# renmengye/rec-attend-public

Hardware: AMD Instinct MI355X
Metric: instance-timesteps/sec, full_model forward 512x512 T=16 (whole job; pipelined throughput: 8 batches in flight per GPU, fill and drain of the pipeline inside the timed region; config.lone_batch_* = one sync-bracketed forward) (higher is better)
Workload: dtype f32; 1 GPU; cfg2: CVPPP-arch full_model eval forward, 512x512, T=16, B=8 per GPU, y_out+s_out; arch=cvppp, H=512, W=512, T=16, batch_per_gpu=8, global_batch=8, parallelism=batch-sharded x1, no collective, ranks_in_communicator=1, hip_graph=True, tile_tickets=False, batches_in_flight=8, pipeline_slots=4, batches_per_launch=2, input=resident in HBM, output=left in HBM

## Files before the change

### rec-attend-public_amd/csrc/ra_ctrl_split.hip

```cpp
#include <cstdlib>
#include <type_traits>

#include "ra_common.h"
#include "ra_ctrl_parts.h"

namespace ra {
namespace ctrl2 {

typedef float f32x4 __attribute__((ext_vector_type(4)));
typedef unsigned long long u64;

constexpr int kP = 16;
constexpr int kThreads = 256;
constexpr int kMaxFeatRegs = 96;
constexpr unsigned kSpinLimit = 4000000u;
constexpr int kMaxResidentWgs = 224;

struct Layout {
  int us, gs, K, NL;
  size_t lstm_w, lstm_b;
  size_t gh_w[8], gh_b[8];
  size_t gl_w, gl_b;
  size_t slice;
  size_t cmlp;
  size_t cm_w[8], cm_b[8];
  int cm_in[8], cm_out[8];
  size_t total;
  int n_hidden;
};

__host__ __device__ inline Layout layout(const ra_ctrl_desc &d) {
  Layout L;
  L.us = d.hid / kP;
  L.gs = ceil_div(d.G, kP);
  L.K = d.Cf + d.hid;
  L.NL = 4 * L.us;
  L.n_hidden = d.n_gmlp - 1;
  size_t off = 0;
  L.lstm_w = off;
  off += (size_t)L.K * L.NL;
  L.lstm_b = off;
  off += L.NL;
  for (int l = 0; l < L.n_hidden; ++l) {
    L.gh_w[l] = off;
    off += (size_t)d.hid * L.us;
    L.gh_b[l] = off;
    off += L.us;
  }
  L.gl_w = off;
  off += (size_t)d.hid * L.gs;
  L.gl_b = off;
  off += L.gs;
  L.slice = round_up((int)off, 4);
  off = L.slice * kP;
  L.cmlp = off;
  for (int l = 0; l < d.n_cmlp; ++l) {
    L.cm_in[l] = (l == 0) ? d.hid : d.mlp_dim;
    L.cm_out[l] = (l == d.n_cmlp - 1) ? 9 : d.mlp_dim;
    L.cm_w[l] = off;
    off += (size_t)L.cm_in[l] * L.cm_out[l];
    L.cm_b[l] = off;
    off += L.cm_out[l];
  }
  L.total = off;
  return L;
}

__host__ __device__ inline size_t granules_per_image(const ra_ctrl_desc &d) {
  const Layout L = layout(d);
  return (size_t)d.iters * (d.hid + (size_t)L.n_hidden * d.hid + (size_t)kP * L.gs);
}
__host__ __device__ inline size_t ws_words_per_image(const ra_ctrl_desc &d) {
  return 2 + 2 * granules_per_image(d);
}

__host__ inline size_t lds_bytes(const ra_ctrl_desc &d) {
  const Layout L = layout(d);
  return (L.slice + 4 * (size_t)kThreads + round_up(L.K, 4) + d.hid + round_up(kP * L.gs, 4) + 64) * sizeof(float);
}

__host__ inline int supported(const ra_ctrl_desc &d) {
  if (d.hid % kP || d.hid > kThreads || d.Cf <= 0 || kThreads % d.Cf || d.n_gmlp < 1 ||
      d.n_gmlp > 8 || d.n_cmlp < 1 || d.n_cmlp > 8 || d.G <= 0 || d.G > 4096 || d.iters <= 0 ||
      d.mlp_dim > kThreads)
    return 0;
  if (kThreads % (d.hid / kP) || kThreads % (4 * (d.hid / kP))) return 0;
  if ((size_t)d.G * d.Cf > (size_t)kMaxFeatRegs * kThreads) return 0;
  if (4 * layout(d).us > kThreads) return 0;
  return lds_bytes(d) <= 160 * 1024;
}

typedef unsigned u32x2g __attribute__((ext_vector_type(2)));
template <bool XL>
struct Exchange {
  u64 *gran;
  __amdgpu_buffer_rsrc_t rs;
  unsigned tag;
  int err = 0;

  __device__ __forceinline__ Exchange(unsigned *wsb, size_t granules)
      : gran(reinterpret_cast<u64 *>(wsb + 2)),
        rs(__builtin_amdgcn_make_buffer_rsrc(gran, 0, (int)(granules * 8), 0x00020000)),
        tag(wsb[0] + 1u) {}

  __device__ __forceinline__ void publish(size_t idx, float v) const {
    if constexpr (XL)
      __builtin_amdgcn_raw_buffer_store_b64(u32x2g{__float_as_uint(v), tag}, rs, (int)idx * 8, 0, 0);
    else
      __hip_atomic_store(gran + idx, ((u64)tag << 32) | (u64)__float_as_uint(v), __ATOMIC_RELAXED, __HIP_MEMORY_SCOPE_AGENT);
  }

  __device__ __forceinline__ u32x2g load(size_t idx) const {
    if constexpr (XL) {
      return __builtin_amdgcn_raw_buffer_load_b64(rs, (int)idx * 8, 0, (int)0x80000001u);
    } else {
      const u64 x = __hip_atomic_load(gran + idx, __ATOMIC_RELAXED, __HIP_MEMORY_SCOPE_AGENT);
      return u32x2g{(unsigned)x, (unsigned)(x >> 32)};
    }
  }

  template <int INFLIGHT, class Store>
  __device__ __forceinline__ void poll(size_t first, int total, Store store) {
    for (int base = 0; base < total; base += kThreads * INFLIGHT) {
      unsigned pending = 0;
#pragma unroll
      for (int j = 0; j < INFLIGHT; ++j)
        if (base + threadIdx.x + kThreads * j < total) pending |= 1u << j;
      unsigned spins = 0;
      while (pending) {
        u32x2g x[INFLIGHT];
#pragma unroll
        for (int j = 0; j < INFLIGHT; ++j)
          if (pending & (1u << j)) x[j] = load(first + base + threadIdx.x + kThreads * j);
#pragma unroll
        for (int j = 0; j < INFLIGHT; ++j)
          if ((pending & (1u << j)) && x[j].y == tag) {
            store(base + threadIdx.x + kThreads * j, __uint_as_float(x[j].x));
            pending &= ~(1u << j);
          }
        if (pending) {
          if (++spins > kSpinLimit) {
            err = 1;
            break;
          }
          __builtin_amdgcn_s_sleep(1);
        }
      }
    }
    __syncthreads();
  }

  template <int INFLIGHT>
  __device__ __forceinline__ void gather(size_t first, int n, int nimg, float *dst, int stride) {
    poll<INFLIGHT>(first, n * nimg, [&](int e, float v) {
      const int i = e / n, c = e - i * n;
      dst[i * stride + c] = v;
    });
  }
};

__device__ __forceinline__ void fill_slice(float *W, const float *__restrict__ wp, int p, const Layout &L) {
  const int t = threadIdx.x;
  const f32x4 *src = reinterpret_cast<const f32x4 *>(wp + (size_t)p * L.slice);
  f32x4 *dst = reinterpret_cast<f32x4 *>(W);
  const int n4 = (int)(L.slice / 4);
  constexpr int U = 16;
  for (int e0 = t; e0 < n4; e0 += kThreads * U) {
    f32x4 tmp[U];
#pragma unroll
    for (int u = 0; u < U; ++u) {
      const int e = e0 + u * kThreads;
      tmp[u] = src[e < n4 ? e : n4 - 1];
    }
#pragma unroll
    for (int u = 0; u < U; ++u) {
      const int e = e0 + u * kThreads;
      if (e < n4) dst[e] = tmp[u];
    }
  }
}

__device__ float block_reduce(float v, bool is_max, float *red4) {
#pragma unroll
  for (int o = 32; o > 0; o >>= 1) {
    const float other = __shfl_xor(v, o);
    v = is_max ? fmaxf(v, other) : v + other;
  }
  __syncthreads();
  if ((threadIdx.x & 63) == 0) red4[threadIdx.x >> 6] = v;
  __syncthreads();
  const float a = red4[0], b = red4[1], c = red4[2], d = red4[3];
  return is_max ? fmaxf(fmaxf(a, b), fmaxf(c, d)) : (a + b) + (c + d);
}

__device__ inline void slice_gemv(const float *W, int ncol, const float *x, int k0, int K, float *red) {
  const int t = threadIdx.x;
  const int parts = kThreads / ncol;
  const int col = t % ncol, part = t / ncol;
  float acc0 = 0.0f, acc1 = 0.0f;
  int k = k0 + part;
#pragma unroll 4
  for (; k + parts < K; k += 2 * parts) {
    acc0 += x[k] * W[(size_t)k * ncol + col];
    acc1 += x[k + parts] * W[(size_t)(k + parts) * ncol + col];
  }
  if (k < K) acc0 += x[k] * W[(size_t)k * ncol + col];
  red[part * ncol + col] = acc0 + acc1;
  __syncthreads();
}

__device__ inline int any_gemv(const float *Wm, int n, const float *x, int K, float *red, int *ncol_out) {
  const int t = threadIdx.x;
  int ncol = 1;
  while (ncol < n) ncol <<= 1;
  const int parts = kThreads / ncol;
  const int col = t % ncol, part = t / ncol;
  float acc = 0.0f;
  if (col < n)
    for (int k = part; k < K; k += parts) acc += x[k] * Wm[(size_t)k * n + col];
  red[part * ncol + col] = acc;
  __syncthreads();
  *ncol_out = ncol;
  return parts;
}

__device__ __forceinline__ void finish_image(const ra_ctrl_desc &d, const Layout &L, const float *__restrict__ wp, const float *h,
                                             float *o1, float *o2, float *scratch, int b, float *h_last, float *ctrl_out,
                                             float *attn) {
  const int t = threadIdx.x;
  const float *in = h;
  for (int l = 0; l < d.n_cmlp; ++l) {
    const int N = L.cm_out[l], Kin = L.cm_in[l];
    const float *Wc = wp + L.cm_w[l], *bc = wp + L.cm_b[l];
    const bool last = (l == d.n_cmlp - 1);
    int ncol;
    const int parts = any_gemv(Wc, N, in, Kin, scratch, &ncol);
    if (t < N) {
      float a = bc[t];
      for (int q = 0; q < parts; ++q) a += scratch[q * ncol + t];
      o1[t] = last ? a : fmaxf(a, 0.0f);
    }
    __syncthreads();
    in = o1;
    float *tmp = o1;
    o1 = o2;
    o2 = tmp;
  }
  const float *co = in;
  if (t < d.hid && h_last) h_last[(size_t)b * d.hid + t] = h[t];
  if (t < 9 && ctrl_out) ctrl_out[(size_t)b * 9 + t] = co[t];
  if (t == 0 && attn) store_attn_record(d, co, attn + (size_t)b * RA_ATTN_STRIDE);
}

__device__ inline void publish(u64 *g, unsigned tag, float v) {
  __hip_atomic_store(g, ((u64)tag << 32) | (u64)__float_as_uint(v), __ATOMIC_RELAXED,
                     __HIP_MEMORY_SCOPE_AGENT);
}

__device__ inline void gather(const u64 *g, int n, unsigned tag, float *dst, int *err) {
  for (int i = threadIdx.x; i < n; i += kThreads) {
    unsigned spins = 0;
    u64 x;
    while (true) {
      x = __hip_atomic_load(g + i, __ATOMIC_RELAXED, __HIP_MEMORY_SCOPE_AGENT);
      if ((unsigned)(x >> 32) == tag) break;
      if (++spins > kSpinLimit) {
        *err = 1;
        break;
      }
      __builtin_amdgcn_s_sleep(1);
    }
    dst[i] = __uint_as_float((unsigned)x);
  }
  __syncthreads();
}

__device__ inline void publish_l2(__amdgpu_buffer_rsrc_t r, int idx, unsigned tag, float v) {
  __builtin_amdgcn_raw_buffer_store_b64(u32x2g{__float_as_uint(v), tag}, r, idx * 8, 0, 0);
}
__device__ inline void gather_l2(__amdgpu_buffer_rsrc_t r, int first, int n, unsigned tag, float *dst, int *err) {
  for (int i = threadIdx.x; i < n; i += kThreads) {
    unsigned spins = 0;
    u32x2g x;
    while (true) {
      x = __builtin_amdgcn_raw_buffer_load_b64(r, (first + i) * 8, 0, (int)0x80000001u);
      if (x.y == tag) break;
      if (++spins > kSpinLimit) {
        *err = 1;
        break;
      }
      __builtin_amdgcn_s_sleep(1);
    }
    dst[i] = __uint_as_float(x.x);
  }
  __syncthreads();
}

template <int FR, bool XL = false>
__global__ __launch_bounds__(kThreads) void controller_split_kernel(
    const ra_ctrl_desc d, const float *feat, const float *__restrict__ wp, float *h_last,
    float *ctrl_out, float *gmaps, float *attn, unsigned *ws, int *status, int prio, int B, unsigned *tickets) {
  raise_prio(prio);
  extern __shared__ __attribute__((aligned(16))) float smem[];
  const Layout L = layout(d);
  const int t = threadIdx.x;
  int p = blockIdx.x, b = blockIdx.y;
  if constexpr (XL) {
    unsigned *role_sh = reinterpret_cast<unsigned *>(smem);
    const int x = xcc_id(), share = kP * ((B + 7) >> 3);
    if (t == 0) *role_sh = ticket_draw(tickets + x * kTicketPoolStride) % (unsigned)share;
    __syncthreads();
    const int role = (int)*role_sh;
    __syncthreads();
    p = role % kP;
    b = x + 8 * (role / kP);
    if (b >= B) return;
  }
  const int G = d.G, Cf = d.Cf, hid = d.hid, us = L.us, gs = L.gs, K = L.K;
  const int Gx = kP * gs;
  float *W = smem;
  float *red = W + L.slice;
  float *xh = red + 4 * kThreads;
  float *va = xh + round_up(K, 4);
  float *gm = va + hid;
  float *red4 = gm + round_up(Gx, 4);
  unsigned *wsb = ws + (size_t)b * ws_words_per_image(d);
  const unsigned tag = wsb[0] + 1u;
  u64 *gran = reinterpret_cast<u64 *>(wsb + 2);
  const __amdgpu_buffer_rsrc_t grs = __builtin_amdgcn_make_buffer_rsrc(gran, 0, (int)(granules_per_image(d) * 8), 0x00020000);
  int err = 0;
  auto pub = [&](size_t idx, float v) {
    if constexpr (XL) publish_l2(grs, (int)idx, tag, v);
    else publish(gran + idx, tag, v);
  };
  auto gat = [&](size_t first, int n, float *dst) {
    if constexpr (XL) gather_l2(grs, (int)first, n, tag, dst, &err);
    else gather(gran + first, n, tag, dst, &err);
  };

  {
    const f32x4 *src = reinterpret_cast<const f32x4 *>(wp + (size_t)p * L.slice);
    f32x4 *dst = reinterpret_cast<f32x4 *>(W);
    const int n4 = (int)(L.slice / 4);
    constexpr int U = 16;
    for (int e0 = t; e0 < n4; e0 += kThreads * U) {
      f32x4 tmp[U];
#pragma unroll
      for (int u = 0; u < U; ++u) {
        const int e = e0 + u * kThreads;
        tmp[u] = src[e < n4 ? e : n4 - 1];
      }
#pragma unroll
      for (int u = 0; u < U; ++u) {
        const int e = e0 + u * kThreads;
        if (e < n4) dst[e] = tmp[u];
      }
    }
  }
  float fr[FR];
  const float *fsrc = feat + (size_t)b * G * Cf;
#pragma unroll
  for (int i = 0; i < FR; ++i) {
    const int e = t + kThreads * i;
    fr[i] = (e < G * Cf) ? fsrc[e] : 0.0f;
  }
  for (int e = t; e < hid; e += kThreads) xh[Cf + e] = 0.0f;
  for (int g = t; g < Gx; g += kThreads) gm[g] = (g < G) ? 1.0f / (float)G : 0.0f;
  float cst = 0.0f;
  __syncthreads();

  size_t goff = 0;
  for (int it = 0; it < d.iters; ++it) {
    if (gmaps && p == 0)
      for (int g = t; g < G; g += kThreads) gmaps[((size_t)b * d.iters + it) * G + g] = gm[g];
    {
      const int g0 = t / Cf, gstep = kThreads / Cf;
      float s = 0.0f;
#pragma unroll
      for (int i = 0; i < FR; ++i) {
        const int g = g0 + gstep * i;
        s += fr[i] * ((g < G) ? gm[g] : 0.0f);
      }
      red[t] = s;
      __syncthreads();
      if (t < Cf) {
        float a = 0.0f;
        for (int q = 0; q < gstep; ++q) a += red[q * Cf + t];
        xh[t] = a;
      }
      __syncthreads();
    }
    slice_gemv(W + L.lstm_w, L.NL, xh, 0, (it == 0) ? Cf : K, red);
    if (t < us) {
      const int parts = kThreads / L.NL;
      float pre[4];
#pragma unroll
      for (int g = 0; g < 4; ++g) {
        float a = W[L.lstm_b + g * us + t];
        for (int q = 0; q < parts; ++q) a += red[q * L.NL + g * us + t];
        pre[g] = a;
      }
      const float gi = sigm(pre[0]), gf = sigm(pre[1]), go = sigm(pre[2]), u = tanhf(pre[3]);
      cst = gf * cst + gi * u;
      pub(goff + p * us + t, go * tanhf(cst));
    }
    gat(goff, hid, xh + Cf);
    goff += hid;
    if (it == d.iters - 1) break;
    const float *in = xh + Cf;
    for (int l = 0; l < L.n_hidden; ++l) {
      slice_gemv(W + L.gh_w[l], us, in, 0, hid, red);
      if (t < us) {
        const int parts = kThreads / us;
        float a = W[L.gh_b[l] + t];
        for (int q = 0; q < parts; ++q) a += red[q * us + t];
        pub(goff + p * us + t, fmaxf(a, 0.0f));
      }
      gat(goff, hid, va);
      goff += hid;
      in = va;
    }
    {
      int ncol;
      const int parts = any_gemv(W + L.gl_w, gs, in, hid, red, &ncol);
      if (t < gs) {
        float a = W[L.gl_b + t];
        for (int q = 0; q < parts; ++q) a += red[q * ncol + t];
        pub(goff + p * gs + t, a);
      }
      gat(goff, Gx, gm);
      goff += Gx;
      float mx = -3.0e38f;
      for (int g = t; g < G; g += kThreads) mx = fmaxf(mx, gm[g]);
      mx = block_reduce(mx, true, red4);
      float sum = 0.0f;
      for (int g = t; g < G; g += kThreads) sum += expf(gm[g] - mx);
      sum = block_reduce(sum, false, red4);
      __syncthreads();
      for (int g = t; g < Gx; g += kThreads) gm[g] = (g < G) ? expf(gm[g] - mx) / sum : 0.0f;
      __syncthreads();
    }
  }

  if (p == 0) {
    const float *in = xh + Cf;
    float *o1 = va, *o2 = gm;
    for (int l = 0; l < d.n_cmlp; ++l) {
      const int N = L.cm_out[l], Kin = L.cm_in[l];
      const float *Wc = wp + L.cm_w[l], *bc = wp + L.cm_b[l];
      const bool last = (l == d.n_cmlp - 1);
      int ncol;
      const int parts = any_gemv(Wc, N, in, Kin, red, &ncol);
      if (t < N) {
        float a = bc[t];
        for (int q = 0; q < parts; ++q) a += red[q * ncol + t];
        o1[t] = last ? a : fmaxf(a, 0.0f);
      }
      __syncthreads();
      in = o1;
      float *tmp = o1;
      o1 = o2;
      o2 = tmp;
    }
    const float *co = in;
    if (t < hid && h_last) h_last[(size_t)b * hid + t] = xh[Cf + t];
    if (t < 9 && ctrl_out) ctrl_out[(size_t)b * 9 + t] = co[t];
    if (t == 0 && attn) store_attn_record(d, co, attn + (size_t)b * RA_ATTN_STRIDE);
    if (t == 0)
      __hip_atomic_store(wsb, tag, __ATOMIC_RELAXED, __HIP_MEMORY_SCOPE_AGENT);
  }
  if (err && status) atomicMax(status, 1);
}

inline int xcd_local(int *both = nullptr) {
  static int xl = -1, xl_both = 0;
  if (xl < 0) {
    const int asked = env_int("RA_CTRL_XCD", 1);
    xl_both = asked == 2 ? 1 : 0;
    if (asked == 0) xl = 0;
    else if (const int c = xcc_census_ok(); c >= 0) xl = c;
  }
  if (both) *both = xl_both;
  return xl;
}

inline unsigned *ticket_pools(unsigned *ws, size_t ws_bytes) { return ws + ws_bytes / 4 - kTicketSlotWords; }

template <class F>
int with_feat_regs(int fr, F &&f) {
  if (fr <= 4) return f(std::integral_constant<int, 4>());
  if (fr <= 16) return f(std::integral_constant<int, 16>());
  if (fr <= 32) return f(std::integral_constant<int, 32>());
  if (fr <= 64) return f(std::integral_constant<int, 64>());
  return f(std::integral_constant<int, 96>());
}

template <int FR>
int launch(const ra_ctrl_desc &d, const float *feat, const float *wp, int B, float *h_last,
           float *ctrl_out, float *gmaps, float *attn, unsigned *ws, size_t ws_bytes, int *status, hipStream_t st) {
  auto kern = controller_split_kernel<FR, false>;
  auto kern_xl = controller_split_kernel<FR, true>;
  static const MaxDynamicLds lds_limit(kern, 160 * 1024), lds_limit_xl(kern_xl, 160 * 1024);
  const size_t lds = lds_bytes(d);
  unsigned *tickets = ticket_pools(ws, ws_bytes);
  int xl_all;
  const int xl = xcd_local(&xl_all);
  if (xl == 1 && (B <= 8 || xl_all))
    hipLaunchKernelGGL(kern_xl, dim3(8 * kP * ((B + 7) / 8)), dim3(kThreads), lds, st, d, feat, wp, h_last, ctrl_out, gmaps, attn, ws,
                       status, tail_prio(1), B, tickets);
  else
    hipLaunchKernelGGL(kern, dim3(kP, B), dim3(kThreads), lds, st, d, feat, wp, h_last, ctrl_out,
                       gmaps, attn, ws, status, tail_prio(1), B, tickets);
  return launch_status("ra_controller_split_f32");
}

template <int NI>
__host__ __device__ inline size_t granules_per_group(const ra_ctrl_desc &d) {
  const Layout L = layout(d);
  return (size_t)d.iters * NI * (d.Cf + d.hid + (size_t)L.n_hidden * d.hid + (size_t)kP * L.gs);
}
template <int NI>
__host__ __device__ inline size_t ws_words_per_group(const ra_ctrl_desc &d) { return 2 + 2 * granules_per_group<NI>(d); }

template <int NI>
__host__ inline size_t batch_lds_bytes(const ra_ctrl_desc &d) {
  const Layout L = layout(d);
  return (L.slice + (size_t)kThreads * NI + (size_t)NI * round_up(L.K, 4) + (size_t)NI * d.hid +
          (size_t)NI * round_up(kP * L.gs, 4) + 64) * sizeof(float);
}

template <int NI>
__host__ inline int batch_supported(const ra_ctrl_desc &d) {
  if (!supported(d)) return 0;
  const Layout L = layout(d);
  int gsp = 1;
  while (gsp < L.gs) gsp <<= 1;
  if (gsp > 64 || L.us * NI > kThreads || d.Cf > kThreads) return 0;
  return batch_lds_bytes<NI>(d) <= 160 * 1024;
}

template <int NI>
__device__ inline int gemv_multi(const float *W, int n, int ncol, const float *x, int xs, int K, float *red) {
  const int t = threadIdx.x, parts = kThreads / ncol;
  const int col = t % ncol, part = t / ncol;
  float acc[NI];
#pragma unroll
  for (int i = 0; i < NI; ++i) acc[i] = 0.0f;
  if (col < n) {
    const int K4 = K & ~3;
    for (int k = 4 * part; k < K4; k += 4 * parts) {
      const float w0 = W[(size_t)k * n + col], w1 = W[(size_t)(k + 1) * n + col], w2 = W[(size_t)(k + 2) * n + col],
                  w3 = W[(size_t)(k + 3) * n + col];
#pragma unroll
      for (int i = 0; i < NI; ++i) {
        const f32x4 xv = *reinterpret_cast<const f32x4 *>(x + i * xs + k);
        acc[i] += xv.x * w0 + xv.y * w1 + xv.z * w2 + xv.w * w3;
      }
    }
    if (part == 0)
      for (int k = K4; k < K; ++k) {
        const float w = W[(size_t)k * n + col];
#pragma unroll
        for (int i = 0; i < NI; ++i) acc[i] += x[i * xs + k] * w;
      }
  }
#pragma unroll
  for (int i = 0; i < NI; ++i) red[(part * NI + i) * ncol + col] = acc[i];
  __syncthreads();
  return parts;
}

template <int FR, int NI, bool XL = false>
__global__ __launch_bounds__(kThreads) void controller_batch_kernel(const ra_ctrl_desc d, const float *feat,
                                                                    const float *__restrict__ wp, int B, float *h_last,
                                                                    float *ctrl_out, float *gmaps, float *attn,
                                                                    unsigned *ws, int *status, int prio, unsigned *tickets, int xcd_off) {
  raise_prio(prio);
  extern __shared__ __attribute__((aligned(16))) float smem[];
  const Layout L = layout(d);
  const int t = threadIdx.x;
  int p = blockIdx.x, grp = blockIdx.y;
  if constexpr (XL) {
    unsigned *role_sh = reinterpret_cast<unsigned *>(smem);
    const int x = xcc_id();
    if (t == 0) *role_sh = ticket_draw(tickets + x * kTicketPoolStride) % (unsigned)kP;
    __syncthreads();
    p = (int)*role_sh;
    __syncthreads();
    grp = (x - xcd_off) & 7;
    if (grp * NI >= B) return;
  }
  const int G = d.G, Cf = d.Cf, hid = d.hid, us = L.us, gs = L.gs, K = L.K;
  const int Gx = kP * gs, Kp = round_up(K, 4), Gxp = round_up(Gx, 4);
  const int b0 = grp * NI, nimg = (B - b0 < NI) ? B - b0 : NI;
  float *W = smem;
  float *red = W + L.slice;
  float *xh = red + kThreads * NI;
  float *va = xh + NI * Kp;
  float *gm = va + NI * hid;
  unsigned *wsg = ws + (size_t)grp * ws_words_per_group<NI>(d);
  Exchange<XL> ex(wsg, granules_per_group<NI>(d));

  fill_slice(W, wp, p, L);
  const int mine = p % nimg;
  float fr[FR];
  const float *fsrc = feat + (size_t)(b0 + mine) * G * Cf;
#pragma unroll
  for (int i = 0; i < FR; ++i) {
    const int e = t + kThreads * i;
    fr[i] = (e < G * Cf) ? fsrc[e] : 0.0f;
  }
  for (int e = t; e < NI * Kp; e += kThreads) xh[e] = 0.0f;
  for (int e = t; e < NI * Gxp; e += kThreads) gm[e] = ((e % Gxp) < G) ? 1.0f / (float)G : 0.0f;
  float cst = 0.0f;
  const int ci = t / us, cu = t % us;
  __syncthreads();

  size_t goff = 0;
  for (int it = 0; it < d.iters; ++it) {
    if (gmaps && p == 0)
      for (int e = t; e < nimg * G; e += kThreads) {
        const int i = e / G, g = e - i * G;
        gmaps[((size_t)(b0 + i) * d.iters + it) * G + g] = gm[i * Gxp + g];
      }
    {
      const int g0 = t / Cf, gstep = kThreads / Cf;
      const float *gmm = gm + mine * Gxp;
      float s = 0.0f;
#pragma unroll
      for (int i = 0; i < FR; ++i) {
        const int g = g0 + gstep * i;
        s += fr[i] * ((g < G) ? gmm[g] : 0.0f);
      }
      red[t] = s;
      __syncthreads();
      if (t < Cf && p < nimg) {
        float a = 0.0f;
        for (int q = 0; q < gstep; ++q) a += red[q * Cf + t];
        ex.publish(goff + (size_t)mine * Cf + t, a);
      }
      __syncthreads();
    }
    ex.template gather<8>(goff, Cf, nimg, xh, Kp);
    goff += (size_t)NI * Cf;
    {
      const int parts = gemv_multi<NI>(W + L.lstm_w, L.NL, L.NL, xh, Kp, (it == 0) ? Cf : K, red);
      if (t < us * NI && ci < nimg) {
        float pre[4];
#pragma unroll
        for (int g = 0; g < 4; ++g) {
          float a = W[L.lstm_b + g * us + cu];
          for (int q = 0; q < parts; ++q) a += red[(q * NI + ci) * L.NL + g * us + cu];
          pre[g] = a;
        }
        const float gi = sigm(pre[0]), gf = sigm(pre[1]), go = sigm(pre[2]), u = tanhf(pre[3]);
        cst = gf * cst + gi * u;
        ex.publish(goff + (size_t)ci * hid + p * us + cu, go * tanhf(cst));
      }
    }
    ex.template gather<8>(goff, hid, nimg, xh + Cf, Kp);
    goff += (size_t)NI * hid;
    if (it == d.iters - 1) break;
    const float *in = xh + Cf;
    int ins = Kp;
    for (int l = 0; l < L.n_hidden; ++l) {
      const int parts = gemv_multi<NI>(W + L.gh_w[l], us, us, in, ins, hid, red);
      if (t < us * NI && ci < nimg) {
        float a = W[L.gh_b[l] + cu];
        for (int q = 0; q < parts; ++q) a += red[(q * NI + ci) * us + cu];
        ex.publish(goff + (size_t)ci * hid + p * us + cu, fmaxf(a, 0.0f));
      }
      ex.template gather<8>(goff, hid, nimg, va, hid);
      goff += (size_t)NI * hid;
      in = va;
      ins = hid;
    }
    {
      int ncol = 1;
      while (ncol < gs) ncol <<= 1;
      const int parts = gemv_multi<NI>(W + L.gl_w, gs, ncol, in, ins, hid, red);
      const int li = t / ncol, lu = t % ncol;
      if (t < ncol * NI && li < nimg && lu < gs) {
        float a = W[L.gl_b + lu];
        for (int q = 0; q < parts; ++q) a += red[(q * NI + li) * ncol + lu];
        ex.publish(goff + (size_t)li * Gx + p * gs + lu, a);
      }
      ex.template gather<8>(goff, Gx, nimg, gm, Gxp);
      goff += (size_t)NI * Gx;
      const int wave = t >> 6, lane = t & 63;
      for (int i = wave; i < nimg; i += kThreads / 64) {
        float *gi = gm + i * Gxp;
        float mx = -3.0e38f;
        for (int g = lane; g < G; g += 64) mx = fmaxf(mx, gi[g]);
        for (int o = 32; o > 0; o >>= 1) mx = fmaxf(mx, __shfl_xor(mx, o));
        float sum = 0.0f;
        for (int g = lane; g < G; g += 64) sum += expf(gi[g] - mx);
        for (int o = 32; o > 0; o >>= 1) sum += __shfl_xor(sum, o);
        for (int g = lane; g < Gx; g += 64) gi[g] = (g < G) ? expf(gi[g] - mx) / sum : 0.0f;
      }
      __syncthreads();
    }
  }

  if (p < nimg) finish_image(d, L, wp, xh + p * Kp + Cf, va + p * hid, red, red + 2 * kThreads, b0 + p, h_last, ctrl_out, attn);
  if (p == 0 && t == 0) __hip_atomic_store(wsg, ex.tag, __ATOMIC_RELAXED, __HIP_MEMORY_SCOPE_AGENT);
  if (ex.err && status) atomicMax(status, 1);
}

template <int FR, int NI>
int launch_batch(const ra_ctrl_desc &d, const float *feat, const float *wp, int B, float *h_last, float *ctrl_out,
                 float *gmaps, float *attn, unsigned *ws, size_t ws_bytes, int *status, int xcd_off, hipStream_t st) {
  auto kern = controller_batch_kernel<FR, NI, false>;
  auto kern_xl = controller_batch_kernel<FR, NI, true>;
  static const MaxDynamicLds lds_limit(kern, 160 * 1024), lds_limit_xl(kern_xl, 160 * 1024);
  const size_t lds = batch_lds_bytes<NI>(d);
  unsigned *tickets = ticket_pools(ws, ws_bytes);
  const int xl = xcd_local();
  if (xl == 1 && xcd_off >= 0 && ceil_div(B, NI) <= 8)
    hipLaunchKernelGGL(kern_xl, dim3(8 * kP), dim3(kThreads), lds, st, d, feat, wp, B, h_last, ctrl_out, gmaps, attn, ws, status,
                       tail_prio(1), tickets, xcd_off & 7);
  else
    hipLaunchKernelGGL(kern, dim3(kP, ceil_div(B, NI)), dim3(kThreads), lds, st, d, feat, wp, B, h_last, ctrl_out, gmaps,
                       attn, ws, status, tail_prio(1), tickets, 0);
  return launch_status("ra_controller_batch_f32");
}

inline int group_images(const ra_ctrl_desc &d, int B) { return (B > 8 && batch_supported<8>(d)) ? 8 : 4; }

}
}

using namespace ra;

extern "C" int ra_ctrl_split_supported(const ra_ctrl_desc *d) { return d ? ctrl2::supported(*d) : 0; }

extern "C" size_t ra_ctrl_split_packed_floats(const ra_ctrl_desc *d) {
  if (!d || !ctrl2::supported(*d)) return 0;
  return ctrl2::layout(*d).total;
}

extern "C" size_t ra_ctrl_split_workspace_bytes(const ra_ctrl_desc *d, int B) {
  if (!d || B <= 0 || !ctrl2::supported(*d)) return 0;
  return ((size_t)B * ctrl2::ws_words_per_image(*d) + kTicketSlotWords) * 4;
}

extern "C" int ra_ctrl_split_pack_weights(const ra_ctrl_desc *d, const float *const *lstm_w,
                                          const float *const *gmlp_w, const float *const *cmlp_w,
                                          float *out) {
  if (!d || !lstm_w || !gmlp_w || !cmlp_w || !out || !ctrl2::supported(*d))
    return fail(RA_E_SHAPE, "ra_ctrl_split_pack_weights: unsupported descriptor / null argument");
  const ctrl2::Layout L = ctrl2::layout(*d);
  const int Cf = d->Cf, hid = d->hid, us = L.us, gs = L.gs;
  for (size_t i = 0; i < L.total; ++i) out[i] = 0.0f;
  const int gate_of_ref[4] = {0, 1, 3, 2};
  for (int p = 0; p < ctrl2::kP; ++p) {
    float *S = out + (size_t)p * L.slice;
    for (int r = 0; r < 4; ++r) {
      const float *wx = lstm_w[3 * r], *wh = lstm_w[3 * r + 1], *bb = lstm_w[3 * r + 2];
      const int g = gate_of_ref[r];
      for (int u = 0; u < us; ++u) {
        const int j = p * us + u, col = g * us + u;
        for (int k = 0; k < Cf; ++k) S[L.lstm_w + (size_t)k * L.NL + col] = wx[(size_t)k * hid + j];
        for (int k = 0; k < hid; ++k) S[L.lstm_w + (size_t)(Cf + k) * L.NL + col] = wh[(size_t)k * hid + j];
        S[L.lstm_b + col] = bb[j];
      }
    }
    for (int l = 0; l < L.n_hidden; ++l) {
      const float *ww = gmlp_w[2 * l], *bb = gmlp_w[2 * l + 1];
      for (int u = 0; u < us; ++u) {
        for (int k = 0; k < hid; ++k) S[L.gh_w[l] + (size_t)k * us + u] = ww[(size_t)k * hid + p * us + u];
        S[L.gh_b[l] + u] = bb[p * us + u];
      }
    }
    const float *ww = gmlp_w[2 * L.n_hidden], *bb = gmlp_w[2 * L.n_hidden + 1];
    for (int u = 0; u < gs; ++u) {
      const int g = p * gs + u;
      if (g >= d->G) continue;
      for (int k = 0; k < hid; ++k) S[L.gl_w + (size_t)k * gs + u] = ww[(size_t)k * d->G + g];
      S[L.gl_b + u] = bb[g];
    }
  }
  for (int l = 0; l < d->n_cmlp; ++l) {
    const float *ww = cmlp_w[2 * l], *bb = cmlp_w[2 * l + 1];
    for (size_t i = 0; i < (size_t)L.cm_in[l] * L.cm_out[l]; ++i) out[L.cm_w[l] + i] = ww[i];
    for (int i = 0; i < L.cm_out[l]; ++i) out[L.cm_b[l] + i] = bb[i];
  }
  return 0;
}

extern "C" int ra_controller_split_f32(const ra_ctrl_desc *d, const float *feat, const float *wpacked,
                                       int B, float *h_last, float *ctrl_out, float *glimpse_maps,
                                       float *attn, void *ws, size_t ws_bytes, int *status_dev,
                                       void *stream) {
  if (!d || !feat || !wpacked || !ws || B <= 0) return fail(RA_E_INVALID, "ra_controller_split_f32: bad argument");
  if (!ctrl2::supported(*d)) return fail(RA_E_SHAPE, "ra_controller_split_f32: unsupported descriptor");
  if (B * ctrl2::kP > ctrl2::kMaxResidentWgs) return fail(RA_E_SHAPE, "ra_controller_split_f32: B=%d exceeds co-residency (%d)", B,
                                                                  ctrl2::kMaxResidentWgs / ctrl2::kP);
  if (ws_bytes < ra_ctrl_split_workspace_bytes(d, B)) return fail(RA_E_WORKSPACE, "ra_controller_split_f32: workspace");
  unsigned *w = reinterpret_cast<unsigned *>(ws);
  return ctrl2::with_feat_regs(ceil_div(d->G * d->Cf, ctrl2::kThreads), [&](auto FR) {
    return ctrl2::launch<decltype(FR)::value>(*d, feat, wpacked, B, h_last, ctrl_out, glimpse_maps, attn, w, ws_bytes, status_dev,
                                              as_stream(stream));
  });
}

extern "C" int ra_ctrl_batch_supported(const ra_ctrl_desc *d) { return d ? ctrl2::batch_supported<4>(*d) : 0; }

extern "C" int ra_ctrl_batch_group_images(const ra_ctrl_desc *d, int B) {
  if (!d || B <= 0 || !ctrl2::batch_supported<4>(*d)) return 0;
  return ctrl2::group_images(*d, B);
}

extern "C" size_t ra_ctrl_batch_workspace_bytes(const ra_ctrl_desc *d, int B) {
  if (!d || B <= 0 || !ctrl2::batch_supported<4>(*d)) return 0;
  const int g = ctrl2::group_images(*d, B);
  return ((size_t)ceil_div(B, g) * (g == 8 ? ctrl2::ws_words_per_group<8>(*d) : ctrl2::ws_words_per_group<4>(*d)) + kTicketSlotWords) * 4;
}

extern "C" int ra_controller_batch_f32(const ra_ctrl_desc *d, const float *feat, const float *wpacked, int B,
                                       float *h_last, float *ctrl_out, float *glimpse_maps, float *attn, void *ws,
                                       size_t ws_bytes, int *status_dev, void *stream) {
  return ra_controller_batch_xcd_f32(d, feat, wpacked, B, h_last, ctrl_out, glimpse_maps, attn, ws, ws_bytes, status_dev, -1, stream);
}

extern "C" int ra_controller_batch_xcd_f32(const ra_ctrl_desc *d, const float *feat, const float *wpacked, int B,
                                           float *h_last, float *ctrl_out, float *glimpse_maps, float *attn, void *ws,
                                           size_t ws_bytes, int *status_dev, int xcd_offset, void *stream) {
  if (!d || !feat || !wpacked || !ws || B <= 0) return fail(RA_E_INVALID, "ra_controller_batch_f32: bad argument");
  if (!ctrl2::batch_supported<4>(*d)) return fail(RA_E_SHAPE, "ra_controller_batch_f32: unsupported descriptor");
  const int g = ctrl2::group_images(*d, B);
  if (ceil_div(B, g) * ctrl2::kP > ctrl2::kMaxResidentWgs)
    return fail(RA_E_SHAPE, "ra_controller_batch_f32: B=%d exceeds co-residency (%d)", B, ctrl2::kMaxResidentWgs / ctrl2::kP * g);
  if (ws_bytes < ra_ctrl_batch_workspace_bytes(d, B)) return fail(RA_E_WORKSPACE, "ra_controller_batch_f32: workspace");
  unsigned *w = reinterpret_cast<unsigned *>(ws);
  return ctrl2::with_feat_regs(ceil_div(d->G * d->Cf, ctrl2::kThreads), [&](auto FR) {
    constexpr int fr = decltype(FR)::value;
    hipStream_t st = as_stream(stream);
    return g == 8 ? ctrl2::launch_batch<fr, 8>(*d, feat, wpacked, B, h_last, ctrl_out, glimpse_maps, attn, w, ws_bytes, status_dev, xcd_offset, st)
                  : ctrl2::launch_batch<fr, 4>(*d, feat, wpacked, B, h_last, ctrl_out, glimpse_maps, attn, w, ws_bytes, status_dev, xcd_offset, st);
  });
}
```

Before: 62040 instance-timesteps/s.

## Slim controller batch kernel: compact offsets, fused softmax, fma gemv, probe hooks

Replaces the array-heavy Layout struct in the batch controller kernel with a small set of computed integer offsets, which should lower register and scalar pressure. The softmax now gives each image its own lane group (a wave or half-wave), caches the exponentials in place and skips recomputing them. The gemv inner loop uses chained fmaf, and the feature dot product clamps the index instead of branching. Optional phase-probe hooks are added but compile out by default. The main risk is that the recomputed offsets may not match the host packing of weights.

```diff
diff --git a/rec-attend-public_amd/csrc/ra_ctrl_split.hip b/rec-attend-public_amd/csrc/ra_ctrl_split.hip
--- a/rec-attend-public_amd/csrc/ra_ctrl_split.hip
+++ b/rec-attend-public_amd/csrc/ra_ctrl_split.hip
@@ -159,11 +159,11 @@
   }
 };
 
-__device__ __forceinline__ void fill_slice(float *W, const float *__restrict__ wp, int p, const Layout &L) {
+__device__ __forceinline__ void fill_slice(float *W, const float *__restrict__ wp, int p, int slice) {
   const int t = threadIdx.x;
-  const f32x4 *src = reinterpret_cast<const f32x4 *>(wp + (size_t)p * L.slice);
+  const f32x4 *src = reinterpret_cast<const f32x4 *>(wp + (size_t)p * slice);
   f32x4 *dst = reinterpret_cast<f32x4 *>(W);
-  const int n4 = (int)(L.slice / 4);
+  const int n4 = slice / 4;
   constexpr int U = 16;
   for (int e0 = t; e0 < n4; e0 += kThreads * U) {
     f32x4 tmp[U];
@@ -224,15 +224,16 @@
   return parts;
 }
 
-__device__ __forceinline__ void finish_image(const ra_ctrl_desc &d, const Layout &L, const float *__restrict__ wp, const float *h,
+__device__ __forceinline__ void finish_image(const ra_ctrl_desc &d, size_t cmlp, const float *__restrict__ wp, const float *h,
                                              float *o1, float *o2, float *scratch, int b, float *h_last, float *ctrl_out,
                                              float *attn) {
   const int t = threadIdx.x;
   const float *in = h;
+  const float *Wc = wp + cmlp;
   for (int l = 0; l < d.n_cmlp; ++l) {
-    const int N = L.cm_out[l], Kin = L.cm_in[l];
-    const float *Wc = wp + L.cm_w[l], *bc = wp + L.cm_b[l];
     const bool last = (l == d.n_cmlp - 1);
+    const int N = last ? 9 : d.mlp_dim, Kin = (l == 0) ? d.hid : d.mlp_dim;
+    const float *bc = Wc + (size_t)Kin * N;
     int ncol;
     const int parts = any_gemv(Wc, N, in, Kin, scratch, &ncol);
     if (t < N) {
@@ -241,6 +242,7 @@
       o1[t] = last ? a : fmaxf(a, 0.0f);
     }
     __syncthreads();
+    Wc = bc + N;
     in = o1;
     float *tmp = o1;
     o1 = o2;
@@ -516,8 +518,7 @@
 
 template <int NI>
 __host__ __device__ inline size_t granules_per_group(const ra_ctrl_desc &d) {
-  const Layout L = layout(d);
-  return (size_t)d.iters * NI * (d.Cf + d.hid + (size_t)L.n_hidden * d.hid + (size_t)kP * L.gs);
+  return (size_t)d.iters * NI * (d.Cf + d.hid + (size_t)(d.n_gmlp - 1) * d.hid + (size_t)kP * ceil_div(d.G, kP));
 }
 template <int NI>
 __host__ __device__ inline size_t ws_words_per_group(const ra_ctrl_desc &d) { return 2 + 2 * granules_per_group<NI>(d); }
@@ -540,7 +541,7 @@
 }
 
 template <int NI>
-__device__ inline int gemv_multi(const float *W, int n, int ncol, const float *x, int xs, int K, float *red) {
+__device__ inline void gemv_multi(const float *W, int n, int ncol, const float *x, int xs, int K, float *red) {
   const int t = threadIdx.x, parts = kThreads / ncol;
   const int col = t % ncol, part = t / ncol;
   float acc[NI];
@@ -554,7 +555,7 @@
 #pragma unroll
       for (int i = 0; i < NI; ++i) {
         const f32x4 xv = *reinterpret_cast<const f32x4 *>(x + i * xs + k);
-        acc[i] += xv.x * w0 + xv.y * w1 + xv.z * w2 + xv.w * w3;
+        acc[i] = fmaf(xv.w, w3, fmaf(xv.z, w2, fmaf(xv.y, w1, fmaf(xv.x, w0, acc[i]))));
       }
     }
     if (part == 0)
@@ -567,8 +568,38 @@
 #pragma unroll
   for (int i = 0; i < NI; ++i) red[(part * NI + i) * ncol + col] = acc[i];
   __syncthreads();
-  return parts;
-}
+}
+
+template <int NI>
+__device__ __forceinline__ float add_parts(float a, const float *red, int ncol, int i, int c) {
+  for (int q = 0; q < kThreads / ncol; ++q) a += red[(q * NI + i) * ncol + c];
+  return a;
+}
+
+struct GroupOffs {
+  int us, gs, K, NL, lstm_b, gh0, ghs, gl_w, gl_b, slice;
+};
+__host__ __device__ inline GroupOffs group_offs(const ra_ctrl_desc &d) {
+  GroupOffs o;
+  o.us = d.hid / kP;
+  o.gs = ceil_div(d.G, kP);
+  o.K = d.Cf + d.hid;
+  o.NL = 4 * o.us;
+  o.lstm_b = o.K * o.NL;
+  o.gh0 = o.lstm_b + o.NL;
+  o.ghs = d.hid * o.us + o.us;
+  o.gl_w = o.gh0 + (d.n_gmlp - 1) * o.ghs;
+  o.gl_b = o.gl_w + d.hid * o.gs;
+  o.slice = round_up(o.gl_b + o.gs, 4);
+  return o;
+}
+
+#ifdef RA_PROBE_CTRLB
+__device__ long long *ra_probe_ctrlb_buf;
+#define RA_PHASE_PROBE_BUF ra_probe_ctrlb_buf
+#define RA_PHASE_PROBE_WG (blockIdx.y * gridDim.x + blockIdx.x)
+#endif
+#include "ra_phase_probe.h"
 
 template <int FR, int NI, bool XL = false>
 __global__ __launch_bounds__(kThreads) void controller_batch_kernel(const ra_ctrl_desc d, const float *feat,
@@ -576,8 +607,9 @@
                                                                     float *ctrl_out, float *gmaps, float *attn,
                                                                     unsigned *ws, int *status, int prio, unsigned *tickets, int xcd_off) {
   raise_prio(prio);
+  RA_PHASE_DECL;
   extern __shared__ __attribute__((aligned(16))) float smem[];
-  const Layout L = layout(d);
+  const GroupOffs L = group_offs(d);
   const int t = threadIdx.x;
   int p = blockIdx.x, grp = blockIdx.y;
   if constexpr (XL) {
@@ -601,7 +633,7 @@
   unsigned *wsg = ws + (size_t)grp * ws_words_per_group<NI>(d);
   Exchange<XL> ex(wsg, granules_per_group<NI>(d));
 
-  fill_slice(W, wp, p, L);
+  fill_slice(W, wp, p, L.slice);
   const int mine = p % nimg;
   float fr[FR];
   const float *fsrc = feat + (size_t)(b0 + mine) * G * Cf;
@@ -615,6 +647,7 @@
   float cst = 0.0f;
   const int ci = t / us, cu = t % us;
   __syncthreads();
+  RA_PHASE_AT(0);
 
   size_t goff = 0;
   for (int it = 0; it < d.iters; ++it) {
@@ -630,7 +663,7 @@
 #pragma unroll
       for (int i = 0; i < FR; ++i) {
         const int g = g0 + gstep * i;
-        s += fr[i] * ((g < G) ? gmm[g] : 0.0f);
+        s += fr[i] * gmm[g < G ? g : G - 1];
       }
       red[t] = s;
       __syncthreads();
@@ -641,36 +674,36 @@
       }
       __syncthreads();
     }
+    RA_PHASE_AT(1);
     ex.template gather<8>(goff, Cf, nimg, xh, Kp);
+    RA_PHASE_AT(2);
     goff += (size_t)NI * Cf;
     {
-      const int parts = gemv_multi<NI>(W + L.lstm_w, L.NL, L.NL, xh, Kp, (it == 0) ? Cf : K, red);
+      gemv_multi<NI>(W, L.NL, L.NL, xh, Kp, (it == 0) ? Cf : K, red);
       if (t < us * NI && ci < nimg) {
         float pre[4];
 #pragma unroll
-        for (int g = 0; g < 4; ++g) {
-          float a = W[L.lstm_b + g * us + cu];
-          for (int q = 0; q < parts; ++q) a += red[(q * NI + ci) * L.NL + g * us + cu];
-          pre[g] = a;
-        }
+        for (int g = 0; g < 4; ++g) pre[g] = add_parts<NI>(W[L.lstm_b + g * us + cu], red, L.NL, ci, g * us + cu);
         const float gi = sigm(pre[0]), gf = sigm(pre[1]), go = sigm(pre[2]), u = tanhf(pre[3]);
         cst = gf * cst + gi * u;
         ex.publish(goff + (size_t)ci * hid + p * us + cu, go * tanhf(cst));
       }
     }
+    RA_PHASE_AT(3);
     ex.template gather<8>(goff, hid, nimg, xh + Cf, Kp);
+    RA_PHASE_AT(2);
     goff += (size_t)NI * hid;
     if (it == d.iters - 1) break;
     const float *in = xh + Cf;
     int ins = Kp;
-    for (int l = 0; l < L.n_hidden; ++l) {
-      const int parts = gemv_multi<NI>(W + L.gh_w[l], us, us, in, ins, hid, red);
-      if (t < us * NI && ci < nimg) {
-        float a = W[L.gh_b[l] + cu];
-        for (int q = 0; q < parts; ++q) a += red[(q * NI + ci) * us + cu];
-        ex.publish(goff + (size_t)ci * hid + p * us + cu, fmaxf(a, 0.0f));
-      }
+    for (int l = 0; l < d.n_gmlp - 1; ++l) {
+      const float *Wl = W + L.gh0 + l * L.ghs;
+      gemv_multi<NI>(Wl, us, us, in, ins, hid, red);
+      if (t < us * NI && ci < nimg)
+        ex.publish(goff + (size_t)ci * hid + p * us + cu, fmaxf(add_parts<NI>(Wl[hid * us + cu], red, us, ci, cu), 0.0f));
+      RA_PHASE_AT(4);
       ex.template gather<8>(goff, hid, nimg, va, hid);
+      RA_PHASE_AT(2);
       goff += (size_t)NI * hid;
       in = va;
       ins = hid;
@@ -678,33 +711,40 @@
     {
       int ncol = 1;
       while (ncol < gs) ncol <<= 1;
-      const int parts = gemv_multi<NI>(W + L.gl_w, gs, ncol, in, ins, hid, red);
+      gemv_multi<NI>(W + L.gl_w, gs, ncol, in, ins, hid, red);
       const int li = t / ncol, lu = t % ncol;
-      if (t < ncol * NI && li < nimg && lu < gs) {
-        float a = W[L.gl_b + lu];
-        for (int q = 0; q < parts; ++q) a += red[(q * NI + li) * ncol + lu];
-        ex.publish(goff + (size_t)li * Gx + p * gs + lu, a);
-      }
+      if (t < ncol * NI && li < nimg && lu < gs)
+        ex.publish(goff + (size_t)li * Gx + p * gs + lu, add_parts<NI>(W[L.gl_b + lu], red, ncol, li, lu));
+      RA_PHASE_AT(4);
       ex.template gather<8>(goff, Gx, nimg, gm, Gxp);
+      RA_PHASE_AT(2);
       goff += (size_t)NI * Gx;
-      const int wave = t >> 6, lane = t & 63;
-      for (int i = wave; i < nimg; i += kThreads / 64) {
-        float *gi = gm + i * Gxp;
-        float mx = -3.0e38f;
-        for (int g = lane; g < G; g += 64) mx = fmaxf(mx, gi[g]);
-        for (int o = 32; o > 0; o >>= 1) mx = fmaxf(mx, __shfl_xor(mx, o));
-        float sum = 0.0f;
-        for (int g = lane; g < G; g += 64) sum += expf(gi[g] - mx);
-        for (int o = 32; o > 0; o >>= 1) sum += __shfl_xor(sum, o);
-        for (int g = lane; g < Gx; g += 64) gi[g] = (g < G) ? expf(gi[g] - mx) / sum : 0.0f;
-      }
+      constexpr int LPI = kThreads / NI;
+      static_assert(LPI == 32 || LPI == 64, "an image's lanes are a wave or half of one");
+      const int si = t / LPI, sl = t % LPI;
+      const int gend = (si < nimg) ? G : 0, gxend = (si < nimg) ? Gx : 0;
+      float *gi = gm + si * Gxp;
+      float mx = -3.0e38f;
+      for (int g = sl; g < gend; g += LPI) mx = fmaxf(mx, gi[g]);
+      for (int o = LPI / 2; o > 0; o >>= 1) mx = fmaxf(mx, __shfl_xor(mx, o));
+      float sum = 0.0f;
+      for (int g = sl; g < gend; g += LPI) {
+        const float e = expf(gi[g] - mx);
+        gi[g] = e;
+        sum += e;
+      }
+      for (int o = LPI / 2; o > 0; o >>= 1) sum += __shfl_xor(sum, o);
+      for (int g = sl; g < gxend; g += LPI) gi[g] = (g < G) ? gi[g] / sum : 0.0f;
       __syncthreads();
-    }
-  }
-
-  if (p < nimg) finish_image(d, L, wp, xh + p * Kp + Cf, va + p * hid, red, red + 2 * kThreads, b0 + p, h_last, ctrl_out, attn);
+      RA_PHASE_AT(5);
+    }
+  }
+
+  if (p < nimg) finish_image(d, (size_t)L.slice * kP, wp, xh + p * Kp + Cf, va + p * hid, red, red + 2 * kThreads, b0 + p, h_last, ctrl_out, attn);
   if (p == 0 && t == 0) __hip_atomic_store(wsg, ex.tag, __ATOMIC_RELAXED, __HIP_MEMORY_SCOPE_AGENT);
   if (ex.err && status) atomicMax(status, 1);
+  RA_PHASE_AT(6);
+  RA_PHASE_END;
 }
 
 template <int FR, int NI>
```

New measurement: 61010 instance-timesteps/s. 0.983x the previous value.
